# joezie/Personalized-PageRank-Algorithms-on-Neo4j

Hardware: AMD Instinct MI355X
Metric: single-source PPR queries/sec (FORA, alpha=0.15, eps=0.5) (higher is better)
Workload: dtype f64

## Files before the change

personalized-pagerank-algorithms-on-neo4j_amd/csrc/batch.cpp:

```cpp
#include <algorithm>
#include <chrono>
#include <cstdio>
#include <cstring>
#include <memory>
#include <mutex>
#include <new>
#include <thread>

#include "batch_driver.hpp"

using namespace pprhip;
using namespace pprhip::detail;

namespace pprhip {
namespace detail {

int launch_sweep(pprhip_graph* P, ForaRun* runs, const bool* active, int n_active, SweepTicket* T, const int* ws) {
  BatchState* bs = P->batch;
  const GraphData* D = P->gr;
  T->n_active = n_active;
  int n_seeded = 0;
  for (int s = 0; s < kBatch; ++s) {
    T->ws[s] = (ws && active[s]) ? ws[s] : s;
    pprhip_graph* S = bs->slots[T->ws[s]];
// ... 623 lines not shown
  std::unique_lock<std::mutex> lk(mu);
  for (;;) {
    cv.wait(lk, [&] { return n_workers == 0 || err != 0 || (n_wait > 0 && n_hold == 0); });
    if (n_workers == 0 || err != 0) return;
    sweeping = true;
    bool active[kBatch];
    int n_active = 0;
    for (int s = 0; s < kBatch; ++s) {
      active[s] = waitflag[s];
      n_active += active[s] ? 1 : 0;
    }
    lk.unlock();
    const int rc = run_sweep(P, runs, active, n_active);
    const std::string msg = rc != PPRHIP_OK ? get_error() : "";
    lk.lock();
    if (rc != PPRHIP_OK && !err) {
      err = rc;
      errmsg = msg;
    }
    for (int s = 0; s < kBatch; ++s)
      if (active[s]) {
        waitflag[s] = false;
        n_wait--;
        hold[s] = true;
        n_hold++;
      }
    sweeping = false;
    cv.notify_all();
  }
}

}

int pprhip::detail::batch_run(pprhip_graph_t* g, BatchJob& J, pprhip_stats_t* stats_sum) {
  PPRHIP_TRY(ensure_batch(g));
  if (pushes_backward(J.kind)) PPRHIP_TRY(ensure_bwd_layout(g));
  const int q = J.q;
  const char* env = tuning_env("PPRHIP_BATCH_THREADS");
  const bool threaded = q > 1 && (env ? env[0] == '1' : !is_whole_graph(J.kind));
  std::memset(&J.sum, 0, sizeof J.sum);
  if (J.reserve_out && J.kind != QueryKind::kBackward && q > 1) {
    if (!g->batch->fetch) g->batch->fetch = new (std::nothrow) FetchPipe();
    if (!g->batch->fetch) return PPRHIP_ERR_OOM;
    const int prc = g->batch->fetch->ensure(g);
    if (prc != PPRHIP_OK) {
      g->batch->fetch->destroy();
      delete g->batch->fetch;
      g->batch->fetch = nullptr;
      return prc;
    }
    g->batch->fetch->start();
    J.pipe = g->batch->fetch;
  }
  ForaRun runs[kBatch];
  g->ktimer.stream = g->stream;
  g->ktimer.reset();
  const auto t0 = std::chrono::steady_clock::now();
  share_walks_of(J);
  int rc = PPRHIP_OK;
  double tot[8] = {0};
  uint64_t bytes[8] = {0};
  uint32_t cnt[8] = {0};
  if (threaded) {
    BatchSync B;
    B.P = g;
    B.runs = runs;
// ... 22 lines not shown
      S->c8_via_parent = false;
      S->sync = nullptr;
    }
    KernelTimer local;
    KernelTimer* const saved = g_timer_cur;
    g_timer_cur = &local;
    local.stream = g->stream;
    rc = batch_sequential(J);
    (void)hipStreamSynchronize(g->stream);
    local.resolve(tot, bytes, cnt);
    local.destroy();
    g_timer_cur = saved;
  }
  (void)hipStreamSynchronize(g->stream);
  if (g->batch->share) g->batch->share->on = false;
  if (J.pipe) {
    const std::string msg = rc != PPRHIP_OK ? get_error() : std::string();
    const int prc = J.pipe->finish();
    J.pipe = nullptr;
    if (rc != PPRHIP_OK) set_error("%s", msg.c_str());
    else rc = prc;
  }
  if (rc != PPRHIP_OK) {
    const std::string msg = get_error();
    g->seed_on = false;
    free_batch(g);
    set_error("%s", msg.c_str());
    return rc;
  }
  g->ktimer.resolve(tot, bytes, cnt);
  pprhip_stats_t& sum = J.sum;
  sum.total_ms = std::chrono::duration<double, std::milli>(std::chrono::steady_clock::now() - t0).count();
  fold_class_totals(sum, tot, bytes, cnt);
  if (stats_sum) *stats_sum = sum;
  return PPRHIP_OK;
}
```

personalized-pagerank-algorithms-on-neo4j_amd/csrc/engine.hpp:

```cpp
#pragma once

#include <atomic>
#include <cstdlib>
#include <vector>

#include "common.hpp"

namespace pprhip {

constexpr int kMaxBatch = 8;

struct DevCounters {
  unsigned long long hist[16];
  unsigned long long packed[2];
  double dead[2];
  unsigned long long dead_pops;
  unsigned long long walk_steps;
  unsigned long long walks_total;
  unsigned long long sources_total;
  unsigned long long walk_loads;
  unsigned long long walk_lanes;
  unsigned long long walks_served;
  unsigned long long share_served;
  unsigned long long share_stored;
// ... 365 lines not shown
  int32_t* zin_rows = nullptr;
  uint32_t n_zin = 0;
  unsigned long long* cross_bits = nullptr;
  uint32_t n_src_live = 0;
  uint32_t n_live = 0;
  std::vector<GsBlock> gs_plan;
  int gs_plan_B = 0;
  SlicedLayout* sl = nullptr;
  PanelLayout* pn = nullptr;
  uint8_t* start_flags_o = nullptr;
  uint32_t* chunk_starts_o = nullptr;
  int32_t *nz_rows_o = nullptr, *z_rows_o = nullptr;
  uint32_t n_nz_o = 0, n_z_o = 0;
  unsigned long long* cross_bits_o = nullptr;
  double* survival = nullptr;
  double survival_alpha = 0.0;
  WalkIndex* widx = nullptr;
  double *out_w = nullptr, *out_cum = nullptr, *wsum = nullptr, *in_w = nullptr;
  uint64_t w_bytes = 0;
  double* wsurvival = nullptr;
  double wsurvival_alpha = 0.0;
};

struct BatchState {
  std::vector<pprhip_graph*> slots;
  double* c8[2] = {nullptr, nullptr};
  int c8cur = 0;
  double* acc8 = nullptr;
  int acc8_dir = 0;
  unsigned long long* prep_bits = nullptr;
  uint4* apply_meta[2] = {nullptr, nullptr};
  SlotArgs* d_slot_args = nullptr;
  SlotArgs* h_slot_args = nullptr;
  unsigned long long* sweep_out = nullptr;
  unsigned long long* h_sweep_out = nullptr;
  unsigned long long* blk_pack8 = nullptr;
  double* blk_dead8 = nullptr;
  uint32_t* blk_ndead8 = nullptr;
  int col_owner[kBatch];
  hipStream_t slot_stream = nullptr;
  bool slot_stream_tried = false;
  hipStream_t walk_stream = nullptr;
  bool walk_stream_tried = false;
  void (*idle_hook)(void*) = nullptr;
  void* idle_arg = nullptr;
  int in_c8 = 0;
  detail::FetchPipe* fetch = nullptr;
  WalkShare* share = nullptr;
};

struct ApbsWorkspace {
  char* ws = nullptr;
  uint32_t blocks = 0, cap_t = 0, cap_f = 0;
};

}

struct pprhip_graph {
  pprhip::GraphData* gr = nullptr;
  pprhip::BatchState* batch = nullptr;
  hipStream_t stream = nullptr;
  double* acc_nz = nullptr;
  double* pn_part = nullptr;
  uint32_t* pn_ctr = nullptr;
  pprhip_graph* parent = nullptr;
  int slot_index = -1;
// ... 69 lines not shown
};

namespace pprhip {

int launch_sparse_prepare(pprhip_graph* g, const PushArgs& a, int fbuf, int level, uint64_t nf_upper,
                          unsigned long long dense_thresh, bool scatter_dense, int cbuf, int dead_slot,
                          unsigned long long pk0 = ~0ull);
int launch_sparse_levels_wg(pprhip_graph* g, const pprhip::PushArgs& a, int fbuf0, int first, int last,
                            unsigned long long dense_thresh, unsigned long long wg_cap, int dead_slot,
                            unsigned long long pk0);
int launch_sparse_push(pprhip_graph* g, const PushArgs& a, int fbuf, int level, uint64_t ef_upper,
                       unsigned long long dense_thresh, int dead_slot, unsigned long long pk0 = ~0ull);
int launch_seed_land_sparse(pprhip_graph* g, const PushArgs& a, int fbuf, int level, unsigned long long dense_thresh,
                            int dead_slot, unsigned long long pk0);
int init_kernels_push();

struct DenseLaunch {
  const pprhip::GsBlock* blocks = nullptr;
  int n_blocks = 1;
  const int* state_in = nullptr;
  int state0 = pprhip::kGsJacobi;
  unsigned long long* hist_out = nullptr;
  int* state_out = nullptr;
  unsigned long long dense_thresh = 0, gs_thresh = ~0ull;
};
int launch_dense_level(pprhip_graph* g, const PushArgs& a, int cbuf, int out_slot, int dead_slot,
                       const DenseLaunch& d = DenseLaunch());
namespace detail {
const EdgeWindows* sliced_windows_of(pprhip_graph* g, const GsBlock* blocks, int nb);
}
int init_kernels_dense();

constexpr uint32_t kApplyBlocks8 = 2048;
int launch_dense_level_b8(pprhip_graph* parent, bool backward, const pprhip::GsBlock* blocks = nullptr, int n_blocks = 1);
static inline size_t apply_meta_rows(uint32_t n_rows) { return ((size_t)n_rows / 128 + 2) * 128; }
int launch_build_apply_meta(pprhip_graph* parent, bool backward);
#ifdef PPRHIP_TEST_HOOKS
int launch_sweep_edges_only(pprhip_graph* parent, const pprhip::GsBlock& B);
int launch_count_live_lines(pprhip_graph* P, unsigned long long* d_out);
#endif
int init_kernels_dense_batch();

int launch_compact_prepared(pprhip_graph* g, int cbuf, int out_fbuf, unsigned long long* d_counter, bool backward);
int launch_count_active(pprhip_graph* g, const PushArgs& a, int seed_kind, int out_slot);
int launch_seed_list(pprhip_graph* g, const PushArgs& a, int seed_kind, int out_fbuf, unsigned long long* d_counter,
                     bool write_armed = false);
int launch_seed_dense(pprhip_graph* g, const PushArgs& a, int seed_kind, int cbuf, int out_slot, int dead_slot);
int launch_sum(pprhip_graph* g, const double* x, uint32_t n);
int launch_sum_partial(pprhip_graph* g, const double* x, uint32_t n);
bool old_small_kernels();
inline uint32_t act_n(const pprhip_graph* g) { return g->n_act ? g->n_act : g->gr->n; }
int launch_set_f64(pprhip_graph* g, double* p, uint32_t idx, double value);
int launch_permute_out(pprhip_graph* g, const double* x, double* out);
int launch_seed_init(pprhip_graph* g, int fbuf, bool topk = false);
int launch_seed_clear(pprhip_graph* g, uint32_t count);
int init_kernels_frontier();

int init_kernels_walk();
int init_kernels_select();
int init_kernels_apbs();

int launch_build_walk_rec(pprhip_graph* g);
int init_kernels_host();
int launch_publish(pprhip_graph* g, const void* src, uint32_t n_words, unsigned long long seq);
int launch_clear(pprhip_graph* g, const ClearList& L);
int launch_copy_f64(pprhip_graph* g, const double* src, double* dst, size_t n);
// ... 128 lines not shown
```

personalized-pagerank-algorithms-on-neo4j_amd/csrc/engine_internal.hpp:

```cpp
#pragma once

#include <sys/mman.h>

#include <atomic>
#include <chrono>
#include <condition_variable>
#include <functional>
#include <mutex>
#include <new>
#include <thread>
#include <deque>
#include <string>
#include <vector>

#include "engine.hpp"

struct pprhip_results {
  pprhip_graph* g = nullptr;
  int device = 0;
  int capacity = 0, count = 0;
  double* buf = nullptr;
};

namespace pprhip {
// ... 374 lines not shown
  int32_t* ids_out = nullptr;
  double* vals_out = nullptr;
  int* n_out = nullptr;
  pprhip_stats_t* per_query = nullptr;
  QueryKind kind = QueryKind::kFora;
  PairPlan* pairs = nullptr;
  TargetPlan* targets = nullptr;
  double alpha = 0.0, threshold = 0.0;
  std::vector<Triple>* triples = nullptr;
  pprhip_results* keep = nullptr;
  int keep_first = 0;
  FetchPipe* pipe = nullptr;
  std::vector<SeedTable> sets;
  pprhip_stats_t sum{};
  std::mutex sum_mu;
  std::atomic<int> next_query{0};
};

int ensure_survival(pprhip_graph* g, double alpha);
int survival_jacobi(pprhip_graph* g, double alpha, const char* fn, bool both, bool converged,
                    const std::function<int(const double*, double*, unsigned long long*)>& iter, double** out);
int pair_plan(pprhip_graph_t* g, const int32_t* sources, const int32_t* targets, int q, double eps,
              const pprhip_fora_conf_t* conf, double rmax, uint64_t seed, const double* values_out,
              pprhip_stats_t* stats_sum, const char* fn, bool weighted, PairPlan& pp);
int pair_upload(pprhip_graph* g, PairPlan& pp, int workspaces, int n_events, const char* fn);
int pair_collect(pprhip_graph* g, const PairPlan& pp, double* values_out, pprhip_stats_t& sum, pprhip_stats_t* stats_sum,
                 const char* fn);

int target_plan(pprhip_graph_t* g, const int32_t* targets, const double* weights, const uint64_t* offsets, int q,
                double alpha, double rmax, pprhip_results* keep, int k, const int32_t* ids_out, const double* vals_out,
                pprhip_stats_t* stats_sum, const char* fn, bool weighted, TargetPlan& tp);

int batch_run(pprhip_graph_t* g, BatchJob& J, pprhip_stats_t* stats_sum);

struct TripleStore {
  TripleRec* rec = nullptr;
  unsigned long long count = 0, cap = 0;
  ~TripleStore();
  int reserve(pprhip_graph* g, unsigned long long extra);
  int take_device(pprhip_graph* g, const TripleRec* d_rec, unsigned long long count);
  int take_host(pprhip_graph* g, std::vector<Triple>& more);
};
int all_pair_collect(pprhip_graph_t* g, double alpha, double threshold, uint32_t t_begin, uint32_t t_end,
                     TripleStore& store, pprhip_stats_t& st);
int backward_search_whole(pprhip_graph_t* g, int32_t target_internal, double alpha, double rmax, pprhip_stats_t& st);

int backward_start(pprhip_graph* g, LevelCtx& L, PushArgs& a, int32_t target_internal, double alpha, double rmax,
                   double lone_value, bool* pushing);
int pair_walk_blocks(pprhip_graph* g, const PairPlan& pp, uint32_t lo, uint32_t hi, double* part, bool lone,
                     decltype(&launch_pair_walk) walk, pprhip_stats_t& st);

int index_from_triples(uint32_t n, std::vector<Triple>& tr, int k, pprhip_index_t** out);
int index_from_device(pprhip_graph* g, const TripleRec* rec, unsigned long long count, int k, uint32_t v_lo, uint32_t v_hi,
                      pprhip_index_t** out);
int index_concat(const std::vector<pprhip_index_t*>& parts, pprhip_index_t** out);
int ensure_ring(pprhip_graph* g);

int seed_plan(pprhip_graph* g, const int32_t* seeds, const double* weights, int k, double alpha, const char* fn,
              SeedTable& plan, int set = -1);
int seed_plan_sets(pprhip_graph* g, const int32_t* seeds, const double* weights, const uint64_t* offsets, int q,
                   double alpha, const char* fn, std::vector<SeedTable>& plans);
int seed_upload(pprhip_graph* g, SeedTable& plan);
int seed_start(pprhip_graph* g, LevelCtx& L);
void seed_free(pprhip_graph* g);
struct SeedScope {
  pprhip_graph* g;
// ... 15 lines not shown
```

personalized-pagerank-algorithms-on-neo4j_amd/csrc/graph.cpp:

```cpp
#include <algorithm>
#include <chrono>
#include <cstdio>
#include <cstdlib>
#include <cstring>
#include <memory>
#include <mutex>
#include <new>

#include "engine_internal.hpp"

using namespace pprhip;
using namespace pprhip::detail;

namespace pprhip {
namespace detail {


static std::mutex g_dev_init_mu;
static std::vector<char> g_dev_inited;
int init_device_once(int device) {
  std::lock_guard<std::mutex> lk(g_dev_init_mu);
  if ((size_t)device < g_dev_inited.size() && g_dev_inited[device]) return PPRHIP_OK;
  PPRHIP_TRY(init_kernels_push());
  PPRHIP_TRY(init_kernels_dense());
// ... 247 lines not shown
      if (slots.size() > before) {
        drop_slot(slots.back());
        slots.pop_back();
      }
      return rc;
    }
  }
  PPRHIP_CHECK_HIP(hipStreamSynchronize(P->stream));
  return PPRHIP_OK;
}

static int ensure_apply_meta(pprhip_graph* P, bool backward) {
  BatchState* B = P->batch;
  const GraphData* D = P->gr;
  if (!B || B->apply_meta[backward] || (backward && !D->start_flags_o)) return PPRHIP_OK;
  const uint32_t n_rows = backward ? D->n_nz_o + D->n_z_o : D->n_nz + D->n_zin;
  PPRHIP_TRY(alloc_dev((void**)&B->apply_meta[backward], sizeof(uint4) * apply_meta_rows(n_rows)));
  PPRHIP_TRY(launch_build_apply_meta(P, backward));
  PPRHIP_CHECK_HIP(hipStreamSynchronize(P->stream));
  return PPRHIP_OK;
}

static int build_batch(pprhip_graph* P) {
  BatchState* B = P->batch;
  const size_t n = P->gr->n;
  for (int i = 0; i < 2; ++i) {
    PPRHIP_TRY(alloc_dev((void**)&B->c8[i], sizeof(double) * n * kBatch));
    PPRHIP_CHECK_HIP(hipMemsetAsync(B->c8[i], 0, sizeof(double) * n * kBatch, P->stream));
  }
  PPRHIP_TRY(alloc_dev((void**)&B->acc8, sizeof(double) * (n + 1) * kBatch));
  PPRHIP_CHECK_HIP(hipMemsetAsync(B->acc8, 0, sizeof(double) * (n + 1) * kBatch, P->stream));
  PPRHIP_TRY(alloc_dev((void**)&B->prep_bits, sizeof(unsigned long long) * kBatch * (n / 64 + 2)));
  PPRHIP_CHECK_HIP(hipMemsetAsync(B->prep_bits, 0, sizeof(unsigned long long) * kBatch * (n / 64 + 2), P->stream));
  PPRHIP_TRY(alloc_dev((void**)&B->d_slot_args, sizeof(SlotArgs) * kBatch));
  PPRHIP_TRY(alloc_pinned((void**)&B->h_slot_args, sizeof(SlotArgs) * kBatch, hipHostMallocDefault));
  PPRHIP_TRY(alloc_dev((void**)&B->sweep_out, sizeof(unsigned long long) * kBatch));
  PPRHIP_TRY(alloc_pinned((void**)&B->h_sweep_out, sizeof(unsigned long long) * kBatch, hipHostMallocDefault));
  PPRHIP_TRY(alloc_dev((void**)&B->blk_pack8, sizeof(unsigned long long) * kBatch * kApplyBlocks8));
  PPRHIP_TRY(alloc_dev((void**)&B->blk_dead8, sizeof(double) * kBatch * kApplyBlocks8));
  PPRHIP_TRY(alloc_dev((void**)&B->blk_ndead8, sizeof(uint32_t) * kBatch * kApplyBlocks8));
  PPRHIP_TRY(ensure_apply_meta(P, false));
  PPRHIP_TRY(ensure_apply_meta(P, true));
  for (int s = 0; s < kBatch; ++s) {
    B->col_owner[s] = -1;
    PPRHIP_TRY(make_slot(P, s));
  }
  PPRHIP_CHECK_HIP(hipStreamSynchronize(P->stream));
  return PPRHIP_OK;
}

int ensure_batch(pprhip_graph* P) {
  if (P->batch) return PPRHIP_OK;
  P->batch = new (std::nothrow) BatchState();
  if (!P->batch) return PPRHIP_ERR_OOM;
  const int rc = build_batch(P);
  if (rc != PPRHIP_OK) free_batch(P);
  return rc;
}

void free_batch(pprhip_graph* P) {
  P->ktimer.destroy();
  BatchState* B = P->batch;
  if (!B) return;
  if (B->fetch) {
    B->fetch->destroy();
    delete B->fetch;
  }
  free_walk_share(B);
  if (B->walk_stream) (void)hipStreamDestroy(B->walk_stream);
  if (B->slot_stream) (void)hipStreamDestroy(B->slot_stream);
  for (pprhip_graph* S : B->slots) drop_slot(S);
  void* dev[] = {B->c8[0], B->c8[1], B->acc8, B->prep_bits, B->d_slot_args, B->sweep_out, B->blk_pack8, B->blk_dead8,
                 B->blk_ndead8, B->apply_meta[0], B->apply_meta[1]};
  for (void* p : dev)
    if (p) (void)hipFree(p);
  if (B->h_slot_args) (void)hipHostFree(B->h_slot_args);
  if (B->h_sweep_out) (void)hipHostFree(B->h_sweep_out);
  delete B;
  P->batch = nullptr;
}

int ensure_bwd_layout(pprhip_graph* P) {
  GraphData* D = P->gr;
  if (D->start_flags_o) return ensure_apply_meta(P, true);
  const uint32_t n = D->n;
  const uint64_t m = D->m;
  const std::vector<uint32_t>& rp = D->h_out_rp;
  const size_t n_chunks = ((size_t)m + kChunkPad - 1) / kChunkPad;
  std::vector<uint8_t> flags((n_chunks + 1) * (kChunkPad / 8), 0);
  std::vector<uint32_t> chunk_starts(n_chunks + 1, 0);
  std::vector<int32_t> nz, zr;
  for (uint32_t v = 0; v < n; ++v) {
    if (rp[v + 1] == rp[v]) {
      if (D->h_in_rp[v + 1] > D->h_in_rp[v]) zr.push_back((int32_t)v);
      continue;
    }
    nz.push_back((int32_t)v);
    const uint32_t e = rp[v];
    flags[e >> 3] |= (uint8_t)(1u << (e & 7));
    chunk_starts[(size_t)e / kChunkPad + 1]++;
  }
  for (size_t c = 1; c <= n_chunks; ++c) chunk_starts[c] += chunk_starts[c - 1];
  std::vector<unsigned long long> cross(((size_t)n + 63) / 64 + 1, 0ull);
  for (size_t j = 0; j < nz.size(); ++j) {
    const uint32_t v = (uint32_t)nz[j];
    const uint32_t last = rp[v + 1] - 1;
    if (rp[v] / kChunkPad != last / kChunkPad || (last + 1) % kChunkPad == 0 || (uint64_t)last + 1 == m)
      cross[j >> 6] |= 1ull << (j & 63);
// ... 263 lines not shown
```

personalized-pagerank-algorithms-on-neo4j_amd/csrc/kernels_dense_batch.hip:

```cpp
#include "push_device.hpp"

namespace pprhip {

constexpr int kHotBytes = 128 * 1024;
constexpr int kHotDefaultBytes = 32 * 1024;

template <int G, int K>
__device__ __forceinline__ int group_bcast(int x) {
  return __builtin_amdgcn_ds_swizzle(x, (0x1f & ~(G - 1)) | (K << 5));
}

template <int G>
struct ChunkRegsB {
  int4 ia, ib;
  unsigned long long mask[G / 8];
};

template <int G>
__device__ __forceinline__ ChunkRegsB<G> load_chunk_b(const int32_t* __restrict__ in_ci,
                                                      const unsigned long long* __restrict__ flags64, uint32_t c,
                                                      int lane) {
  const unsigned long long e0 = (unsigned long long)c * kChunkEdges + 8ull * lane;
  const int4* p = reinterpret_cast<const int4*>(in_ci + e0);
  ChunkRegsB<G> r;
// ... 123 lines not shown
      const int pf = __shfl_up(F, d);
      if (lane >= d) {
        if (!F) S += ps;
        F |= pf;
      }
    }
    double carry = __shfl_up(S, G);
    if (lane < G) carry = 0.0;
    const unsigned long long hmask = __ballot(h);
    if (h) {
      const bool nonempty = grp > 0 || (cur.mask[0] & 1ull) == 0;
      if (nonempty && before > 0) {
        const double total = carry + first_seg;
        const bool started_here = (hmask & ((1ull << (grp * G)) - 1ull)) != 0;
        double* dst = &accB[(size_t)(before - 1) * G + s];
        if (started_here)
          *dst = total;
        else
          atomic_add_noret(dst, total);
      }
    }
    if (grp == 64 / G - 1) {
      const uint32_t starts = cs + incl;
      if (starts > 0 && S != 0.0) atomic_add_noret(&accB[(size_t)(starts - 1) * G + s], S);
    }
    cur = nxt;
  }
}

constexpr int kApplyRows = 64;
constexpr int kApplyGroups = 2;
constexpr int kApplyThreads = 512;
constexpr int kSlotsPerWave = kBatch / (kApplyThreads / 64);

template <class T>
__device__ __forceinline__ T __attribute__((address_space(1)))* slot_vec(T* p) {
  return (T __attribute__((address_space(1)))*)p;
}
__device__ __forceinline__ bool take_armed_slot(uint32_t* armed_generic, int32_t u) {
  auto armed = slot_vec(armed_generic);
  const uint32_t bit = 1u << ((uint32_t)u & 31u);
  if (!(armed[(uint32_t)u >> 5] & bit)) return false;
  return (__hip_atomic_fetch_and(&armed[(uint32_t)u >> 5], ~bit, __ATOMIC_RELAXED, __HIP_MEMORY_SCOPE_AGENT) & bit) != 0;
}

constexpr int kApplyPerThread = kApplyRows * kBatch / kApplyThreads;

struct ApplyFlight {
  double v[kApplyGroups][kApplyPerThread];
  uint4 md;
  unsigned long long cw[kApplyGroups];
};
__device__ __forceinline__ void apply_flight(ApplyFlight& f, uint32_t tl0, uint32_t n_nz, const double* acc8,
                                             const uint4* __restrict__ meta,
                                             const unsigned long long* __restrict__ cross_bits, int tid) {
  if (tid < kApplyRows * kApplyGroups) f.md = meta[(size_t)tl0 * kApplyRows + tid];
#pragma unroll
  for (int g = 0; g < kApplyGroups; ++g) {
    const uint32_t tl = tl0 + g;
    f.cw[g] = cross_bits[tl];
#pragma unroll
    for (int i = 0; i < kApplyPerThread; ++i) {
      const uint32_t idx = (uint32_t)i * (uint32_t)kApplyThreads + tid;
      const uint32_t j = tl * kApplyRows + idx / kBatch;
      f.v[g][i] = __builtin_nontemporal_load(&acc8[(size_t)(j < n_nz ? j : 0u) * kBatch + idx % kBatch]);
    }
  }
}

__global__ __launch_bounds__(256) void k_build_apply_meta(const int32_t* __restrict__ nz_rows, uint32_t n_nz,
                                                          const int32_t* __restrict__ z_rows, uint32_t n_z,
                                                          const uint32_t* __restrict__ out_rp,
                                                          const uint32_t* __restrict__ in_rp_bwd, uint4* __restrict__ meta,
                                                          uint32_t n_pad) {
  const uint32_t j = blockIdx.x * 256u + threadIdx.x;
  if (j >= n_pad) return;
  const int32_t u = j < n_nz ? nz_rows[j] : (j < n_nz + n_z ? z_rows[j - n_nz] : -1);
  uint4 r = make_uint4((uint32_t)u, 0u, 0u, 0u);
  if (u >= 0) {
    r.y = out_rp[u + 1] - out_rp[u];
    if (in_rp_bwd) r.z = in_rp_bwd[u + 1] - in_rp_bwd[u];
  }
  meta[j] = r;
}

__global__ __launch_bounds__(kApplyThreads) void k_dense_apply_batch(const uint4* __restrict__ meta, uint32_t n_nz,
                                                            uint32_t n_zin, double* __restrict__ acc8,
                                                            double* __restrict__ c8_cur, double* __restrict__ c8_next,
                                                            uint32_t tile_lo, uint32_t tile_hi, uint32_t gs_mask,
                                                            uint32_t entry_mask,
                                                            const SlotArgs* __restrict__ slots,
                                                            const unsigned long long* __restrict__ cross_bits,
                                                            unsigned long long* __restrict__ prep_bits,
                                                            unsigned long long* __restrict__ blk_pack8,
                                                            double* __restrict__ blk_dead8,
                                                            uint32_t* __restrict__ blk_ndead8, uint32_t part_base,
                                                            uint32_t part_stride) {
  __shared__ double tile[kApplyGroups][kApplyRows][kBatch + 1];
  __shared__ double tile_p[kApplyGroups][kApplyRows][kBatch + 1];
  __shared__ int32_t s_u[kApplyGroups][kApplyRows];
  __shared__ uint32_t s_d[kApplyGroups][kApplyRows];
  __shared__ uint32_t s_din[kApplyGroups][kApplyRows];
  const int tid = threadIdx.x, lane = tid & 63;
  const int w = __builtin_amdgcn_readfirstlane(tid >> 6);
  const uint32_t n_rows = n_nz + n_zin;
  const uint32_t n_tiles = (n_rows + kApplyRows - 1) / kApplyRows;
  SlotArgs a[kSlotsPerWave];
#pragma unroll
  for (int i = 0; i < kSlotsPerWave; ++i) a[i] = slots[w * kSlotsPerWave + i];
  double dead_next[kSlotsPerWave];
  unsigned long long pack[kSlotsPerWave];
  uint32_t ndead[kSlotsPerWave];
#pragma unroll
  for (int i = 0; i < kSlotsPerWave; ++i) {
    dead_next[i] = 0.0;
    pack[i] = 0;
    ndead[i] = 0;
  }
  for (uint32_t tl0 = tile_lo + blockIdx.x * kApplyGroups; tl0 < tile_hi; tl0 += gridDim.x * kApplyGroups) {
    ApplyFlight f;
    apply_flight(f, tl0, n_nz, acc8, meta, cross_bits, tid);
#pragma unroll
    for (int g = 0; g < kApplyGroups; ++g) {
#pragma unroll
      for (int i = 0; i < kApplyPerThread; ++i) {
        const uint32_t idx = (uint32_t)i * (uint32_t)kApplyThreads + tid;
        const uint32_t r = idx / kBatch, s = idx % kBatch;
        const uint32_t j = (tl0 + g) * kApplyRows + r;
        const double v = (tl0 + g < tile_hi && j < n_nz) ? f.v[g][i] : 0.0;
        if (v != 0.0 && ((f.cw[g] >> r) & 1ull)) acc8[(size_t)j * kBatch + s] = 0.0;
        tile[g][r][s] = v;
      }
    }
    if (tid < kApplyRows * kApplyGroups) {
      const uint32_t g = tid / kApplyRows, r = tid % kApplyRows;
      const bool in = tl0 + g < tile_hi;
      s_u[g][r] = in ? (int32_t)f.md.x : -1;
      s_d[g][r] = in ? f.md.y : 0u;
      s_din[g][r] = in ? f.md.z : 0u;
    }
    __syncthreads();
    if (entry_mask) {
      double p[kApplyGroups][kApplyPerThread];
#pragma unroll
      for (int g = 0; g < kApplyGroups; ++g) {
#pragma unroll
        for (int i = 0; i < kApplyPerThread; ++i) {
          const uint32_t idx = (uint32_t)i * (uint32_t)kApplyThreads + tid;
          const int32_t ur = s_u[g][idx / kBatch];
          p[g][i] = c8_cur[(size_t)(ur >= 0 ? ur : 0) * kBatch + idx % kBatch];
        }
      }
#pragma unroll
      for (int g = 0; g < kApplyGroups; ++g) {
#pragma unroll
        for (int i = 0; i < kApplyPerThread; ++i) {
          const uint32_t idx = (uint32_t)i * (uint32_t)kApplyThreads + tid;
          const uint32_t r = idx / kBatch, s = idx % kBatch;
          tile_p[g][r][s] = (s_u[g][r] >= 0 && (entry_mask >> s & 1u)) ? p[g][i] : 0.0;
        }
      }
      __syncthreads();
    }
    int32_t u[kApplyGroups];
    uint32_t d[kApplyGroups], din[kApplyGroups];
    double accv[kApplyGroups][kSlotsPerWave], oldv[kApplyGroups][kSlotsPerWave], rsvv[kApplyGroups][kSlotsPerWave];
    bool live[kApplyGroups][kSlotsPerWave];
#pragma unroll
    for (int g = 0; g < kApplyGroups; ++g) {
      u[g] = s_u[g][lane];
      d[g] = s_d[g][lane];
      din[g] = s_din[g][lane];
#pragma unroll
      for (int i = 0; i < kSlotsPerWave; ++i) {
        double acc = tile[g][lane][w * kSlotsPerWave + i];
        const bool on = a[i].active && u[g] >= 0;
        if (on && a[i].mode != kBackward && u[g] == a[i].src) {
          const double dd = a[i].ctr->dead[a[i].dead_slot];
          if (dd > 0.0) {
            acc += dd;
            a[i].ctr->dead[a[i].dead_slot] = 0.0;
          }
        } else if (a[i].seed_w && a[i].mode != kBackward) {
          const double x = a[i].ctr->dead[a[i].dead_slot];
          if (x > 0.0 && on) {
            const double sw = a[i].seed_w[u[g]];
            if (sw != 0.0) acc += x * sw;
          }
        }
        accv[g][i] = acc;
        live[g][i] = on && acc > 0.0;
      }
    }
#pragma unroll
    for (int g = 0; g < kApplyGroups; ++g) {
#pragma unroll
      for (int i = 0; i < kSlotsPerWave; ++i) {
        oldv[g][i] = live[g][i] ? slot_vec(a[i].res)[u[g]] : 0.0;
        rsvv[g][i] = live[g][i] ? slot_vec(a[i].reserve)[u[g]] : 0.0;
      }
    }
#pragma unroll
    for (int g = 0; g < kApplyGroups; ++g) {
#pragma unroll
      for (int i = 0; i < kSlotsPerWave; ++i) {
        const int s = w * kSlotsPerWave + i;
        double cn = 0.0;
        if (live[g][i] && a[i].mode == kBackward) {
          const double old = oldv[g][i];
          const double nw = old + accv[g][i] / (double)d[g];
          if (!(old > a[i].rmax) && nw > a[i].rmax) {
            slot_vec(a[i].reserve)[u[g]] = rsvv[g][i] + nw * a[i].alpha;
            if (oldv[g][i] != 0.0) slot_vec(a[i].res)[u[g]] = 0.0;
            cn = (1.0 - a[i].alpha) * nw;
            pack[i] += (1ull << kPackShift) | (unsigned long long)din[g];
          } else {
            slot_vec(a[i].res)[u[g]] = nw;
          }
        } else if (live[g][i]) {
          const double old = oldv[g][i];
          const double nw = old + accv[g][i];
          bool crossing = !active_fwd(old, d[g], a[i].rmax) && active_fwd(nw, d[g], a[i].rmax);
          if (a[i].mode == kFwdTopk) {
            if (a[i].rmax < a[i].min_rmax && active_fwd(old, d[g], a[i].rmax)) crossing = take_armed_slot(a[i].armed, u[g]);
            if (active_fwd(nw, d[g], a[i].min_rmax)) slot_vec(a[i].flags)[u[g]] = 1;
          }
          if (crossing) {
            slot_vec(a[i].reserve)[u[g]] = rsvv[g][i] + nw * a[i].alpha;
            if (oldv[g][i] != 0.0) slot_vec(a[i].res)[u[g]] = 0.0;
            if (d[g] == 0) {
              dead_next[i] += nw * (1.0 - a[i].alpha);
              ndead[i]++;
            } else {
              cn = ((1.0 - a[i].alpha) * nw) / (double)d[g];
            }
            pack[i] += (1ull << kPackShift) | (unsigned long long)d[g];
          } else {
            slot_vec(a[i].res)[u[g]] = nw;
          }
        }
        tile[g][lane][s] = cn;
        if (gs_mask >> s & 1u) {
          const int gst = a[i].gs_state;
          tile_p[g][lane][s] = gst == kGsEntry ? tile_p[g][lane][s] + cn : (gst == kGsInPlace ? cn : 0.0);
        }
        const unsigned long long bits = __ballot(cn > 0.0);
        if (lane == 0 && a[i].active && tl0 + g < tile_hi) prep_bits[(size_t)s * n_tiles + tl0 + g] = bits;
      }
    }
    __syncthreads();
#pragma unroll
    for (int g = 0; g < kApplyGroups; ++g) {
#pragma unroll
      for (int i = 0; i < kApplyPerThread; ++i) {
        const uint32_t idx = (uint32_t)i * (uint32_t)kApplyThreads + tid;
        const uint32_t r = idx / kBatch, s = idx % kBatch;
        const int32_t ur = s_u[g][r];
        if (ur >= 0) {
          c8_next[(size_t)ur * kBatch + s] = tile[g][r][s];
          if (gs_mask >> s & 1u) c8_cur[(size_t)ur * kBatch + s] = tile_p[g][r][s];
        }
      }
    }
    __syncthreads();
  }
#pragma unroll
  for (int i = 0; i < kSlotsPerWave; ++i) {
    const double ds = wave_sum_f64(dead_next[i]);
    const unsigned long long ps = wave_sum_u64(pack[i]);
    const unsigned long long nd = wave_sum_u64((unsigned long long)ndead[i]);
    if (lane == 0) {
      const size_t o = (size_t)(w * kSlotsPerWave + i) * part_stride + part_base + blockIdx.x;
      blk_pack8[o] = ps;
      blk_dead8[o] = ds;
      blk_ndead8[o] = (uint32_t)nd;
    }
  }
}

__global__ __launch_bounds__(1024) void k_dense_reduce_batch(const unsigned long long* __restrict__ blk_pack8,
                                                           const double* __restrict__ blk_dead8,
                                                           const uint32_t* __restrict__ blk_ndead8, uint32_t n_blocks,
                                                           uint32_t part_stride,
                                                           const SlotArgs* __restrict__ slots,
                                                           unsigned long long* __restrict__ sweep_out) {
// ... 84 lines not shown
    atomicAdd(&out[1], cs);
  }
}
int launch_count_live_lines(pprhip_graph* P, unsigned long long* d_out) {
  const BatchState* bs = P->batch;
  k_count_live_lines<<<dim3((P->gr->n + 255) / 256), dim3(256), 0, P->stream>>>(bs->c8[bs->c8cur], P->gr->out_rp, P->gr->n,
                                                                              d_out);
  PPRHIP_CHECK_HIP(hipGetLastError());
  return PPRHIP_OK;
}

int launch_sweep_edges_only(pprhip_graph* P, const GsBlock& B) {
  const GraphData* D = P->gr;
  const BatchState* bs = P->batch;
  return launch_dense_edges_bG<kBatch>(P, D->in_ci, D->start_flags, D->chunk_starts, bs->c8[bs->c8cur], bs->acc8, B);
}
#endif

int launch_build_apply_meta(pprhip_graph* P, bool backward) {
  const GraphData* D = P->gr;
  const SweepSide S = sweep_side(D, backward);
  const uint32_t n_pad = (uint32_t)apply_meta_rows(S.n_nz + S.n_z);
  k_build_apply_meta<<<dim3((n_pad + 255) / 256), dim3(256), 0, P->stream>>>(
      S.nz_rows, S.n_nz, S.z_rows, S.n_z, D->out_rp, backward ? D->in_rp : nullptr, P->batch->apply_meta[backward], n_pad);
  PPRHIP_CHECK_HIP(hipGetLastError());
  return PPRHIP_OK;
}

static_assert(kApplyRows * kApplyGroups == 128, "apply_meta_rows (engine.hpp) pads the records to pairs of 64-row tiles");
static_assert(kApplyRows == kTileRows, "launch_compact_prepared (kernels_frontier.hip) finds a slot's prep_bits by kTileRows");

int launch_dense_level_b8(pprhip_graph* P, bool backward, const GsBlock* gs_blocks, int n_gs_blocks) {
  const GraphData* D = P->gr;
  const BatchState* bs = P->batch;
  PPRHIP_CHECK_HIP(hipMemcpyAsync(bs->d_slot_args, bs->h_slot_args, sizeof(SlotArgs) * kBatch, hipMemcpyHostToDevice,
                                  P->stream));
  const SweepSide S = sweep_side(D, backward);
  const uint4* meta = bs->apply_meta[backward];
  if (!meta) {
    set_error("batched sweep: no row records for the %s side", backward ? "backward" : "forward");
    return PPRHIP_ERR_INVALID;
  }
  uint32_t gs_mask = 0, entry_mask = 0;
  for (int s = 0; s < kBatch; ++s)
    if (bs->h_slot_args[s].active) {
      const int st = bs->h_slot_args[s].gs_state;
      if (st == kGsEntry || st == kGsInPlace || st == kGsFlush) gs_mask |= 1u << s;
      if (st == kGsEntry) entry_mask |= 1u << s;
    }
  const uint32_t n_rows = S.n_nz + S.n_z;
  const uint32_t n_tiles = (n_rows + kApplyRows - 1) / kApplyRows;
  const GsBlock whole{0u, S.n_nz, 0ull, (unsigned long long)D->m};
  const bool cut = gs_mask && gs_blocks && n_gs_blocks > 1 && !backward;
  const GsBlock* blocks = cut ? gs_blocks : &whole;
  const int nb = cut ? n_gs_blocks : 1;
  uint32_t part_base = 0;
  for (int b = 0; b < nb; ++b) {
    const GsBlock& B = blocks[b];
    PPRHIP_TRY(launch_dense_edges_bG<kBatch>(P, S.ci, S.start_flags, S.chunk_starts, bs->c8[bs->c8cur], bs->acc8, B));
    const uint32_t t_lo = B.j_lo / kApplyRows;
    const uint32_t t_hi = (b == nb - 1) ? n_tiles : B.j_hi / kApplyRows;
    if (t_hi <= t_lo) continue;
    const uint32_t quota = kApplyBlocks8 / (uint32_t)nb;
    uint32_t grid = std::max(1u, std::min((t_hi - t_lo + kApplyGroups - 1) / kApplyGroups, quota));
    if (const char* e = hook_env("PPRHIP_APPLY_GRID"))
      if (atol(e) > 0) grid = (uint32_t)std::min<long>(grid, atol(e));
    k_dense_apply_batch<<<dim3(grid), dim3(kApplyThreads), 0, P->stream>>>(
          meta, S.n_nz, S.n_z, bs->acc8, bs->c8[bs->c8cur],
          bs->c8[bs->c8cur ^ 1], t_lo, t_hi, b == nb - 1 ? 0u : gs_mask, b == nb - 1 ? 0u : entry_mask, bs->d_slot_args,
          S.cross_bits, bs->prep_bits, bs->blk_pack8, bs->blk_dead8, bs->blk_ndead8, part_base, kApplyBlocks8);
    PPRHIP_CHECK_HIP(hipGetLastError());
    part_base += grid;
  }
  uint32_t seed_dead_max = 0;
  bool seeded = false;
  for (int s = 0; s < kBatch; ++s) {
    const SlotArgs& sa = bs->h_slot_args[s];
    if (sa.active && sa.seed_w && !backward) {
      seeded = true;
      seed_dead_max = std::max(seed_dead_max, sa.seed_n_all - sa.seed_n_live);
    }
  }
  if (seeded) {
    k_seed_land_dense_batch<<<dim3(grid_for(seed_dead_max, 256, 1024), kBatch), dim3(256), 0, P->stream>>>(
        bs->d_slot_args);
    PPRHIP_CHECK_HIP(hipGetLastError());
  }
  k_dense_reduce_batch<<<dim3(kBatch), dim3(1024), 0, P->stream>>>(bs->blk_pack8, bs->blk_dead8, bs->blk_ndead8, part_base,
                                                                   kApplyBlocks8, bs->d_slot_args, bs->sweep_out);
  PPRHIP_CHECK_HIP(hipGetLastError());
  return PPRHIP_OK;
}

int init_kernels_dense_batch() {
  PPRHIP_CHECK_HIP(hipFuncSetAttribute(reinterpret_cast<const void*>(&k_dense_edges_b<true, kBatch>),
                                       hipFuncAttributeMaxDynamicSharedMemorySize, kHotBytes));
  hipFuncAttributes fa;
  PPRHIP_CHECK_HIP(hipFuncGetAttributes(&fa, reinterpret_cast<const void*>(&k_dense_apply_batch)));
  return PPRHIP_OK;
}

}
```

personalized-pagerank-algorithms-on-neo4j_amd/csrc/stream.cpp:

```cpp
#include <chrono>
#include <condition_variable>
#include <deque>
#include <map>
#include <memory>
#include <mutex>
#include <thread>

#include "batch_driver.hpp"

using namespace pprhip;
using namespace pprhip::detail;

namespace {

struct StreamJob : BatchJob {
  std::vector<int32_t> own_srcs;
  uint64_t ticket = 0;
  int finished = 0;
  bool done = false;
  std::chrono::steady_clock::time_point t0;
};

}

// ... 44 lines not shown
    g_timer_cur = saved;
    return;
  }
  SlotDriver& D = *Dp;
  (void)D.open(P, true, true);
  hipStream_t side = D.side;
  long fault_at = -1, started = 0;
  if (const char* fe = hook_env("PPRHIP_STREAM_FAULT_AT")) fault_at = atol(fe);
  bool injected = false;
  D.next = [&](BatchJob** job, int* i) {
    if (fault_at >= 0 && started == fault_at) {
      injected = true;
      return false;
    }
    std::lock_guard<std::mutex> lk(s->mu);
    if (s->pending.empty()) return false;
    StreamJob* J = s->pending.front().get();
    *job = J;
    *i = J->next_query.fetch_add(1);
    if (*i + 1 >= J->q) s->pending.pop_front();
    ++started;
    if (*i == 0) {
      bool idle = true;
      for (int w = 0; w < D.n_ws && idle; ++w) idle = D.runs[w].query < 0;
      if (idle) share_walks_of(*J);
    }
    return true;
  };
  D.done = [&](BatchJob* job) {
    StreamJob* J = static_cast<StreamJob*>(job);
    std::lock_guard<std::mutex> lk(s->mu);
    if (++J->finished == J->q) {
      J->sum.total_ms = std::chrono::duration<double, std::milli>(std::chrono::steady_clock::now() - J->t0).count();
      J->done = true;
      s->cv_done.notify_all();
    }
  };
  const int rc = D.run("query stream", " in the driver thread", [&](int busy) -> int {
    if (injected) {
      set_error("query stream: injected failure before query %ld (PPRHIP_STREAM_FAULT_AT)", fault_at);
      return PPRHIP_ERR_STATE;
    }
    if (busy == 0) {
      std::unique_lock<std::mutex> lk(s->mu);
      s->cv_work.wait(lk, [&] { return s->closing || !s->pending.empty(); });
      if (s->pending.empty()) return SlotDriver::kStop;
    }
    return SlotDriver::kGoOn;
  });
  (void)hipStreamSynchronize(P->stream);
  D.teardown();
  if (P->batch->share) P->batch->share->on = false;
  if (P->batch->walk_stream) (void)hipStreamSynchronize(P->batch->walk_stream);
  if (side && side != P->stream && side != P->batch->walk_stream) (void)hipStreamSynchronize(side);
  if (rc != PPRHIP_OK) stream_fail(s, rc);
  g_timer_cur = saved;
}

int stream_error(pprhip_stream* s, const char* fn) {
  set_error("%s: the stream has failed: %s", fn, s->errmsg.c_str());
  return s->err;
}

}

int pprhip_fora_stream_open(pprhip_graph_t* g, double eps, const pprhip_fora_conf_t* conf, int k,
// ... 155 lines not shown
```

Measured before the change: 438.2.

## Skip zero-in-degree apply tiles and lighten dead-end tiles in batched dense sweep

The batched dense apply kernel now classifies tiles by metadata (all dead-end rows, or rows with no in-edges). On relabeled forward sweeps it processes only tiles below the first zero-in-degree tile, plus a short host-built list of tiles that currently or recently held a source. It also skips reading current mass and residuals for dead-end tiles. The aim is to avoid sweeping rows that can never receive mass, in exchange for host bookkeeping, a larger slot-args upload and correctness that depends on the skipped rows staying zero after the first full sweeps.

```diff
diff --git a/personalized-pagerank-algorithms-on-neo4j_amd/csrc/batch.cpp b/personalized-pagerank-algorithms-on-neo4j_amd/csrc/batch.cpp
--- a/personalized-pagerank-algorithms-on-neo4j_amd/csrc/batch.cpp
+++ b/personalized-pagerank-algorithms-on-neo4j_amd/csrc/batch.cpp
@@ -679,6 +679,20 @@
 
 }
 
+#ifdef PPRHIP_TEST_HOOKS
+int pprhip::detail::take_apply_counts(pprhip_graph* g, pprhip_stats_t& sum) {
+  if (!hook_env("PPRHIP_APPLY_COUNT_RES") || !g->batch || !g->batch->apply_res_count) return PPRHIP_OK;
+  unsigned long long c[3] = {0, 0, 0};
+  PPRHIP_CHECK_HIP(hipMemcpyAsync(c, g->batch->apply_res_count, sizeof c, hipMemcpyDeviceToHost, g->stream));
+  PPRHIP_CHECK_HIP(hipMemsetAsync(g->batch->apply_res_count, 0, sizeof c, g->stream));
+  PPRHIP_CHECK_HIP(hipStreamSynchronize(g->stream));
+  sum.class_bytes[7] = c[0];
+  sum.class_launches[7] = (uint32_t)std::min<unsigned long long>(c[1], 0xffffffffull);
+  sum.class_ms[7] = (double)c[2];
+  return PPRHIP_OK;
+}
+#endif
+
 int pprhip::detail::batch_run(pprhip_graph_t* g, BatchJob& J, pprhip_stats_t* stats_sum) {
   PPRHIP_TRY(ensure_batch(g));
   if (pushes_backward(J.kind)) PPRHIP_TRY(ensure_bwd_layout(g));
@@ -767,6 +781,9 @@
   pprhip_stats_t& sum = J.sum;
   sum.total_ms = std::chrono::duration<double, std::milli>(std::chrono::steady_clock::now() - t0).count();
   fold_class_totals(sum, tot, bytes, cnt);
+#ifdef PPRHIP_TEST_HOOKS
+  PPRHIP_TRY(take_apply_counts(g, sum));
+#endif
   if (stats_sum) *stats_sum = sum;
   return PPRHIP_OK;
 }
diff --git a/personalized-pagerank-algorithms-on-neo4j_amd/csrc/engine.hpp b/personalized-pagerank-algorithms-on-neo4j_amd/csrc/engine.hpp
--- a/personalized-pagerank-algorithms-on-neo4j_amd/csrc/engine.hpp
+++ b/personalized-pagerank-algorithms-on-neo4j_amd/csrc/engine.hpp
@@ -421,6 +421,12 @@
   uint4* apply_meta[2] = {nullptr, nullptr};
   SlotArgs* d_slot_args = nullptr;
   SlotArgs* h_slot_args = nullptr;
+  uint32_t zin_hist[2][kBatch];
+  int zin_hist_n[2] = {0, 0};
+  int zin_full_left = 2;
+#ifdef PPRHIP_TEST_HOOKS
+  unsigned long long* apply_res_count = nullptr;
+#endif
   unsigned long long* sweep_out = nullptr;
   unsigned long long* h_sweep_out = nullptr;
   unsigned long long* blk_pack8 = nullptr;
@@ -556,6 +562,9 @@
 int init_kernels_dense();
 
 constexpr uint32_t kApplyBlocks8 = 2048;
+enum ApplyTileClass : uint32_t { kTilePlain = 0, kTileDeadEnd = 1, kTileNoIn = 2 };
+constexpr uint32_t kApplyListMax = 3 * kBatch;
+static inline size_t slot_args_bytes() { return sizeof(SlotArgs) * kBatch + sizeof(uint32_t) * kApplyListMax; }
 int launch_dense_level_b8(pprhip_graph* parent, bool backward, const pprhip::GsBlock* blocks = nullptr, int n_blocks = 1);
 static inline size_t apply_meta_rows(uint32_t n_rows) { return ((size_t)n_rows / 128 + 2) * 128; }
 int launch_build_apply_meta(pprhip_graph* parent, bool backward);
diff --git a/personalized-pagerank-algorithms-on-neo4j_amd/csrc/engine_internal.hpp b/personalized-pagerank-algorithms-on-neo4j_amd/csrc/engine_internal.hpp
--- a/personalized-pagerank-algorithms-on-neo4j_amd/csrc/engine_internal.hpp
+++ b/personalized-pagerank-algorithms-on-neo4j_amd/csrc/engine_internal.hpp
@@ -430,6 +430,9 @@
                 pprhip_stats_t* stats_sum, const char* fn, bool weighted, TargetPlan& tp);
 
 int batch_run(pprhip_graph_t* g, BatchJob& J, pprhip_stats_t* stats_sum);
+#ifdef PPRHIP_TEST_HOOKS
+int take_apply_counts(pprhip_graph* g, pprhip_stats_t& sum);
+#endif
 
 struct TripleStore {
   TripleRec* rec = nullptr;
diff --git a/personalized-pagerank-algorithms-on-neo4j_amd/csrc/graph.cpp b/personalized-pagerank-algorithms-on-neo4j_amd/csrc/graph.cpp
--- a/personalized-pagerank-algorithms-on-neo4j_amd/csrc/graph.cpp
+++ b/personalized-pagerank-algorithms-on-neo4j_amd/csrc/graph.cpp
@@ -303,8 +303,13 @@
   PPRHIP_CHECK_HIP(hipMemsetAsync(B->acc8, 0, sizeof(double) * (n + 1) * kBatch, P->stream));
   PPRHIP_TRY(alloc_dev((void**)&B->prep_bits, sizeof(unsigned long long) * kBatch * (n / 64 + 2)));
   PPRHIP_CHECK_HIP(hipMemsetAsync(B->prep_bits, 0, sizeof(unsigned long long) * kBatch * (n / 64 + 2), P->stream));
-  PPRHIP_TRY(alloc_dev((void**)&B->d_slot_args, sizeof(SlotArgs) * kBatch));
-  PPRHIP_TRY(alloc_pinned((void**)&B->h_slot_args, sizeof(SlotArgs) * kBatch, hipHostMallocDefault));
+  PPRHIP_TRY(alloc_dev((void**)&B->d_slot_args, slot_args_bytes()));
+  PPRHIP_TRY(alloc_pinned((void**)&B->h_slot_args, slot_args_bytes(), hipHostMallocDefault));
+  std::memset(B->h_slot_args, 0, slot_args_bytes());
+#ifdef PPRHIP_TEST_HOOKS
+  PPRHIP_TRY(alloc_dev((void**)&B->apply_res_count, sizeof(unsigned long long) * 3));
+  PPRHIP_CHECK_HIP(hipMemsetAsync(B->apply_res_count, 0, sizeof(unsigned long long) * 3, P->stream));
+#endif
   PPRHIP_TRY(alloc_dev((void**)&B->sweep_out, sizeof(unsigned long long) * kBatch));
   PPRHIP_TRY(alloc_pinned((void**)&B->h_sweep_out, sizeof(unsigned long long) * kBatch, hipHostMallocDefault));
   PPRHIP_TRY(alloc_dev((void**)&B->blk_pack8, sizeof(unsigned long long) * kBatch * kApplyBlocks8));
@@ -345,6 +350,9 @@
                  B->blk_ndead8, B->apply_meta[0], B->apply_meta[1]};
   for (void* p : dev)
     if (p) (void)hipFree(p);
+#ifdef PPRHIP_TEST_HOOKS
+  if (B->apply_res_count) (void)hipFree(B->apply_res_count);
+#endif
   if (B->h_slot_args) (void)hipHostFree(B->h_slot_args);
   if (B->h_sweep_out) (void)hipHostFree(B->h_sweep_out);
   delete B;
diff --git a/personalized-pagerank-algorithms-on-neo4j_amd/csrc/kernels_dense_batch.hip b/personalized-pagerank-algorithms-on-neo4j_amd/csrc/kernels_dense_batch.hip
--- a/personalized-pagerank-algorithms-on-neo4j_amd/csrc/kernels_dense_batch.hip
+++ b/personalized-pagerank-algorithms-on-neo4j_amd/csrc/kernels_dense_batch.hip
@@ -179,6 +179,13 @@
 constexpr int kApplyGroups = 2;
 constexpr int kApplyThreads = 512;
 constexpr int kSlotsPerWave = kBatch / (kApplyThreads / 64);
+constexpr uint32_t kApplyLean = 1u;
+#ifdef PPRHIP_TEST_HOOKS
+constexpr uint32_t kApplyCountRes = 2u;
+#endif
+constexpr uint32_t kApplyStoreDead = 4u;
+constexpr uint32_t kTileDeadEndStored = 3u;
+static_assert((kTileDeadEnd & 1u) && !(kTilePlain & 1u) && !(kTileNoIn & 1u), "bit 0 of a class says dead end");
 
 template <class T>
 __device__ __forceinline__ T __attribute__((address_space(1)))* slot_vec(T* p) {
@@ -228,6 +235,11 @@
     r.y = out_rp[u + 1] - out_rp[u];
     if (in_rp_bwd) r.z = in_rp_bwd[u + 1] - in_rp_bwd[u];
   }
+  if (!in_rp_bwd) {
+    const bool dead_end = u >= 0 && j < n_nz && r.y == 0u;
+    if (__ballot(dead_end) == ~0ull) r.w = kTileDeadEnd;
+    if (__ballot(j >= n_nz) == ~0ull) r.w = kTileNoIn;
+  }
   meta[j] = r;
 }
 
@@ -242,8 +254,11 @@
                                                             unsigned long long* __restrict__ blk_pack8,
                                                             double* __restrict__ blk_dead8,
                                                             uint32_t* __restrict__ blk_ndead8, uint32_t part_base,
-                                                            uint32_t part_stride) {
+                                                            uint32_t part_stride,
+                                                            const uint32_t* __restrict__ tile_list, uint32_t n_list,
+                                                            uint32_t flags, unsigned long long* res_count) {
   __shared__ double tile[kApplyGroups][kApplyRows][kBatch + 1];
+  __shared__ uint32_t s_cls[kApplyGroups];
   __shared__ double tile_p[kApplyGroups][kApplyRows][kBatch + 1];
   __shared__ int32_t s_u[kApplyGroups][kApplyRows];
   __shared__ uint32_t s_d[kApplyGroups][kApplyRows];
@@ -264,7 +279,11 @@
     pack[i] = 0;
     ndead[i] = 0;
   }
-  for (uint32_t tl0 = tile_lo + blockIdx.x * kApplyGroups; tl0 < tile_hi; tl0 += gridDim.x * kApplyGroups) {
+  const uint32_t pair_trips = tile_hi > tile_lo ? (tile_hi - tile_lo + kApplyGroups - 1) / kApplyGroups : 0u;
+  for (uint32_t trip = blockIdx.x; trip < pair_trips + n_list; trip += gridDim.x) {
+    const bool listed = trip >= pair_trips;
+    const uint32_t tl0 = listed ? tile_list[trip - pair_trips] : tile_lo + trip * kApplyGroups;
+    const uint32_t hi = listed ? tl0 + 1u : tile_hi;
     ApplyFlight f;
     apply_flight(f, tl0, n_nz, acc8, meta, cross_bits, tid);
 #pragma unroll
@@ -274,19 +293,32 @@
         const uint32_t idx = (uint32_t)i * (uint32_t)kApplyThreads + tid;
         const uint32_t r = idx / kBatch, s = idx % kBatch;
         const uint32_t j = (tl0 + g) * kApplyRows + r;
-        const double v = (tl0 + g < tile_hi && j < n_nz) ? f.v[g][i] : 0.0;
+        const double v = (tl0 + g < hi && j < n_nz) ? f.v[g][i] : 0.0;
         if (v != 0.0 && ((f.cw[g] >> r) & 1ull)) acc8[(size_t)j * kBatch + s] = 0.0;
         tile[g][r][s] = v;
       }
     }
     if (tid < kApplyRows * kApplyGroups) {
       const uint32_t g = tid / kApplyRows, r = tid % kApplyRows;
-      const bool in = tl0 + g < tile_hi;
+      const bool in = tl0 + g < hi;
       s_u[g][r] = in ? (int32_t)f.md.x : -1;
       s_d[g][r] = in ? f.md.y : 0u;
       s_din[g][r] = in ? f.md.z : 0u;
+      if (r == 0) {
+        uint32_t c = in ? f.md.w : (uint32_t)kTilePlain;
+        if (c == kTileDeadEnd) c = !(flags & kApplyLean) ? (uint32_t)kTilePlain : ((flags & kApplyStoreDead) ? kTileDeadEndStored : c);
+        s_cls[g] = c;
+      }
     }
     __syncthreads();
+    uint32_t cls[kApplyGroups];
+#pragma unroll
+    for (int g = 0; g < kApplyGroups; ++g) cls[g] = __builtin_amdgcn_readfirstlane(s_cls[g]);
+#ifdef PPRHIP_TEST_HOOKS
+    if ((flags & kApplyCountRes) && entry_mask && tid == 0)
+      for (int g = 0; g < kApplyGroups; ++g)
+        if (cls[g] & 1u) atomicAdd(res_count + 2, 1ull);
+#endif
     if (entry_mask) {
       double p[kApplyGroups][kApplyPerThread];
 #pragma unroll
@@ -295,7 +327,8 @@
         for (int i = 0; i < kApplyPerThread; ++i) {
           const uint32_t idx = (uint32_t)i * (uint32_t)kApplyThreads + tid;
           const int32_t ur = s_u[g][idx / kBatch];
-          p[g][i] = c8_cur[(size_t)(ur >= 0 ? ur : 0) * kBatch + idx % kBatch];
+          p[g][i] = 0.0;
+          if (cls[g] != kTileDeadEnd) p[g][i] = c8_cur[(size_t)(ur >= 0 ? ur : 0) * kBatch + idx % kBatch];
         }
       }
 #pragma unroll
@@ -343,7 +376,14 @@
     for (int g = 0; g < kApplyGroups; ++g) {
 #pragma unroll
       for (int i = 0; i < kSlotsPerWave; ++i) {
-        oldv[g][i] = live[g][i] ? slot_vec(a[i].res)[u[g]] : 0.0;
+        oldv[g][i] = live[g][i] && !(cls[g] & 1u) ? slot_vec(a[i].res)[u[g]] : 0.0;
+#ifdef PPRHIP_TEST_HOOKS
+        if ((flags & kApplyCountRes) && (cls[g] & 1u) && live[g][i]) {
+          oldv[g][i] = slot_vec(a[i].res)[u[g]];
+          atomicAdd(res_count + 1, 1ull);
+          if (oldv[g][i] != 0.0) atomicAdd(res_count, 1ull);
+        }
+#endif
         rsvv[g][i] = live[g][i] ? slot_vec(a[i].reserve)[u[g]] : 0.0;
       }
     }
@@ -391,13 +431,15 @@
           const int gst = a[i].gs_state;
           tile_p[g][lane][s] = gst == kGsEntry ? tile_p[g][lane][s] + cn : (gst == kGsInPlace ? cn : 0.0);
         }
-        const unsigned long long bits = __ballot(cn > 0.0);
-        if (lane == 0 && a[i].active && tl0 + g < tile_hi) prep_bits[(size_t)s * n_tiles + tl0 + g] = bits;
+        const unsigned long long bits = (cls[g] & 1u) ? 0ull : __ballot(cn > 0.0);
+        const bool wr = a[i].active || cls[g] == kTileNoIn;
+        if (lane == 0 && wr && tl0 + g < hi) prep_bits[(size_t)s * n_tiles + tl0 + g] = bits;
       }
     }
     __syncthreads();
 #pragma unroll
     for (int g = 0; g < kApplyGroups; ++g) {
+      if (cls[g] == kTileDeadEnd) continue;
 #pragma unroll
       for (int i = 0; i < kApplyPerThread; ++i) {
         const uint32_t idx = (uint32_t)i * (uint32_t)kApplyThreads + tid;
@@ -548,9 +590,7 @@
 
 int launch_dense_level_b8(pprhip_graph* P, bool backward, const GsBlock* gs_blocks, int n_gs_blocks) {
   const GraphData* D = P->gr;
-  const BatchState* bs = P->batch;
-  PPRHIP_CHECK_HIP(hipMemcpyAsync(bs->d_slot_args, bs->h_slot_args, sizeof(SlotArgs) * kBatch, hipMemcpyHostToDevice,
-                                  P->stream));
+  BatchState* bs = P->batch;
   const SweepSide S = sweep_side(D, backward);
   const uint4* meta = bs->apply_meta[backward];
   if (!meta) {
@@ -570,24 +610,6 @@
   const bool cut = gs_mask && gs_blocks && n_gs_blocks > 1 && !backward;
   const GsBlock* blocks = cut ? gs_blocks : &whole;
   const int nb = cut ? n_gs_blocks : 1;
-  uint32_t part_base = 0;
-  for (int b = 0; b < nb; ++b) {
-    const GsBlock& B = blocks[b];
-    PPRHIP_TRY(launch_dense_edges_bG<kBatch>(P, S.ci, S.start_flags, S.chunk_starts, bs->c8[bs->c8cur], bs->acc8, B));
-    const uint32_t t_lo = B.j_lo / kApplyRows;
-    const uint32_t t_hi = (b == nb - 1) ? n_tiles : B.j_hi / kApplyRows;
-    if (t_hi <= t_lo) continue;
-    const uint32_t quota = kApplyBlocks8 / (uint32_t)nb;
-    uint32_t grid = std::max(1u, std::min((t_hi - t_lo + kApplyGroups - 1) / kApplyGroups, quota));
-    if (const char* e = hook_env("PPRHIP_APPLY_GRID"))
-      if (atol(e) > 0) grid = (uint32_t)std::min<long>(grid, atol(e));
-    k_dense_apply_batch<<<dim3(grid), dim3(kApplyThreads), 0, P->stream>>>(
-          meta, S.n_nz, S.n_z, bs->acc8, bs->c8[bs->c8cur],
-          bs->c8[bs->c8cur ^ 1], t_lo, t_hi, b == nb - 1 ? 0u : gs_mask, b == nb - 1 ? 0u : entry_mask, bs->d_slot_args,
-          S.cross_bits, bs->prep_bits, bs->blk_pack8, bs->blk_dead8, bs->blk_ndead8, part_base, kApplyBlocks8);
-    PPRHIP_CHECK_HIP(hipGetLastError());
-    part_base += grid;
-  }
   uint32_t seed_dead_max = 0;
   bool seeded = false;
   for (int s = 0; s < kBatch; ++s) {
@@ -597,6 +619,69 @@
       seed_dead_max = std::max(seed_dead_max, sa.seed_n_all - sa.seed_n_live);
     }
   }
+  const char* const all_rows_env = hook_env("PPRHIP_APPLY_ALL_ROWS");
+  const bool all_rows = all_rows_env && all_rows_env[0] == '1';
+  const uint32_t z_lo = (S.n_nz + kApplyRows - 1) / kApplyRows;
+  uint32_t now[kBatch];
+  int n_now = 0;
+  auto add_unique = [](uint32_t* v, int& n, uint32_t t) {
+    for (int i = 0; i < n; ++i)
+      if (v[i] == t) return;
+    v[n++] = t;
+  };
+  if (backward || seeded || !D->relabeled) {
+    bs->zin_full_left = 3;
+  } else {
+    for (int s = 0; s < kBatch; ++s) {
+      const SlotArgs& sa = bs->h_slot_args[s];
+      if (!sa.active || sa.src < 0) continue;
+      const uint32_t t = (uint32_t)sa.src / kApplyRows;
+      if (t >= z_lo && t < n_tiles) add_unique(now, n_now, t);
+    }
+  }
+  const bool full = all_rows || bs->zin_full_left > 0;
+  if (bs->zin_full_left > 0) bs->zin_full_left--;
+  uint32_t* list = reinterpret_cast<uint32_t*>(bs->h_slot_args + kBatch);
+  int n_list = 0;
+  if (!full) {
+    for (int i = 0; i < n_now; ++i) add_unique(list, n_list, now[i]);
+    for (int h = 0; h < 2; ++h)
+      for (int i = 0; i < bs->zin_hist_n[h]; ++i) add_unique(list, n_list, bs->zin_hist[h][i]);
+  }
+  std::copy(bs->zin_hist[0], bs->zin_hist[0] + bs->zin_hist_n[0], bs->zin_hist[1]);
+  bs->zin_hist_n[1] = bs->zin_hist_n[0];
+  std::copy(now, now + n_now, bs->zin_hist[0]);
+  bs->zin_hist_n[0] = n_now;
+  PPRHIP_CHECK_HIP(hipMemcpyAsync(bs->d_slot_args, bs->h_slot_args, slot_args_bytes(), hipMemcpyHostToDevice, P->stream));
+  const uint32_t* d_list = reinterpret_cast<const uint32_t*>(bs->d_slot_args + kBatch);
+  uint32_t flags = all_rows ? 0u : (full ? kApplyLean | kApplyStoreDead : kApplyLean);
+  unsigned long long* res_count = nullptr;
+#ifdef PPRHIP_TEST_HOOKS
+  res_count = bs->apply_res_count;
+  if (hook_env("PPRHIP_APPLY_COUNT_RES") && flags) flags |= kApplyCountRes;
+#endif
+  uint32_t part_base = 0;
+  for (int b = 0; b < nb; ++b) {
+    const GsBlock& B = blocks[b];
+    const bool last = b == nb - 1;
+    PPRHIP_TRY(launch_dense_edges_bG<kBatch>(P, S.ci, S.start_flags, S.chunk_starts, bs->c8[bs->c8cur], bs->acc8, B));
+    const uint32_t t_lo = B.j_lo / kApplyRows;
+    const uint32_t t_hi = last ? (full ? n_tiles : z_lo) : B.j_hi / kApplyRows;
+    const uint32_t nl = last && !full ? (uint32_t)n_list : 0u;
+    const uint32_t trips = (t_hi > t_lo ? (t_hi - t_lo + kApplyGroups - 1) / kApplyGroups : 0u) + nl;
+    if (!trips) continue;
+    const uint32_t quota = kApplyBlocks8 / (uint32_t)nb;
+    uint32_t grid = std::max(1u, std::min(trips, quota));
+    if (const char* e = hook_env("PPRHIP_APPLY_GRID"))
+      if (atol(e) > 0) grid = (uint32_t)std::min<long>(grid, atol(e));
+    k_dense_apply_batch<<<dim3(grid), dim3(kApplyThreads), 0, P->stream>>>(
+          meta, S.n_nz, S.n_z, bs->acc8, bs->c8[bs->c8cur],
+          bs->c8[bs->c8cur ^ 1], t_lo, t_hi, last ? 0u : gs_mask, last ? 0u : entry_mask, bs->d_slot_args,
+          S.cross_bits, bs->prep_bits, bs->blk_pack8, bs->blk_dead8, bs->blk_ndead8, part_base, kApplyBlocks8, d_list, nl,
+          flags, res_count);
+    PPRHIP_CHECK_HIP(hipGetLastError());
+    part_base += grid;
+  }
   if (seeded) {
     k_seed_land_dense_batch<<<dim3(grid_for(seed_dead_max, 256, 1024), kBatch), dim3(256), 0, P->stream>>>(
         bs->d_slot_args);
diff --git a/personalized-pagerank-algorithms-on-neo4j_amd/csrc/stream.cpp b/personalized-pagerank-algorithms-on-neo4j_amd/csrc/stream.cpp
--- a/personalized-pagerank-algorithms-on-neo4j_amd/csrc/stream.cpp
+++ b/personalized-pagerank-algorithms-on-neo4j_amd/csrc/stream.cpp
@@ -100,6 +100,9 @@
     std::lock_guard<std::mutex> lk(s->mu);
     if (++J->finished == J->q) {
       J->sum.total_ms = std::chrono::duration<double, std::milli>(std::chrono::steady_clock::now() - J->t0).count();
+#ifdef PPRHIP_TEST_HOOKS
+      (void)take_apply_counts(P, J->sum);
+#endif
       J->done = true;
       s->cv_done.notify_all();
     }
```

Result: faster. 447.3 (median of 6 runs) (+2.1%).
